# well-robotics/Decentralized_EKF_MHE

Measured on AMD Instinct MI355X. Metric: estimator-steps/sec (EKF+MHE, 20-step window), higher is better.
Workload: dtype f64

## Files before the change

### decentralized_ekf_mhe_amd/csrc/cfg.h

```cpp
#pragma once
#include "../../include/dekf.h"
#include "wave.h"

namespace dekf {

#ifndef DEKF_SOLVE_THREADS
#define DEKF_SOLVE_THREADS 256
#endif

#ifndef DEKF_QUEUE_MODE
#define DEKF_QUEUE_MODE 2
#endif
#define DEKF_R4_THREADS 192

constexpr int DEKF_PROF_SLOTS = 32;
constexpr double OSQP_INFTY = 1e30;
constexpr double RHO_MIN = 1e-6, RHO_MAX = 1e6, RHO_EQ_OVER_RHO_INEQ = 1e3, RHO_TOL = 1e-4;
constexpr double MIN_SCALING = 1e-4, MAX_SCALING = 1e4;

struct DevCfg {
    int B, L, nj, N, nm;
    int ft;
    int ns;
    int SV, SC;
    int ring;
    int wcap;
    int rec;
    int snap_len;
    int est_type;
    int marg_info;
    double dt;
    double hdt2, rho0c, inf_thr;
    int gws_wt;
    double C_p[3], C_accel[3], C_accel_bias[3], C_gyro[3];
    double C_enc_pos[DEKF_MAX_JOINTS], C_enc_vel[DEKF_MAX_JOINTS];
    double C_swing[3], Q_swing[3], Q_vo[3], Q_bias_dt2[3];
    double C_slide[3], Q_slide[3];
    double Q_prior[9], C_prior[9];
    double Q_foot_init[3], C_foot_init[3];
    double rho0, sigma, alpha, eps_abs, eps_rel;
    int max_iter, scaling, check_termination, adaptive_rho, adaptive_rho_interval;
    double adaptive_rho_tolerance;
    int polish, polish_refine_iter;
    int polish_accept_osqp;
    double delta;
    double ekf_dt, ekf_Cgyro[3], ekf_Caccel[3], ekf_Cvo[4], ekf_P0[4], ekf_q0[4];
    int ekf_hist;
// ... 75 lines not shown
        cf = o; o += m_pad;
        pol = o; o += 2 * K * ns + 5 * m_pad;
        WT = o; o += wt && !ft ? K * b2 : 0;
        o += wt && !ft ? 8 * 81 : 0;
        total = o;
    }
};

struct DevState {
    double *imu_t, *accel, *gyro, *p_foot, *J, *qdot, *contact, *quat;
    int* vo_flag;
    double *vo_tpre, *vo_tnow, *vo_dp;
    int* ekf_vo_flag;
    double *ekf_vo_t, *ekf_vo_q;
    double *ekf_q, *ekf_P, *ekf_hist;
    double *st_time, *st_R;
    int* st_dtime;
    double *rec, *Mp, *np_;
    double *Mp_next, *np_next;
    int* marg_tag;
    double* snap;
    double *wp, *wpt;
    int* wp_count;
    double* p_vo;
    int *vo_ins_idx, *vo_ins_dtime;
    double* gws;
    int* queue;
    double *kf_x, *kf_C;
    double *x_mhe, *v_b;
    int *status, *iters, *rho_updates;
    int* polish_status;
    double *pri_res, *dua_res;
    double* prof;
    double* warm = nullptr;
    int* warm_tag = nullptr;
    int* warm_used = nullptr;
};

}
```

### decentralized_ekf_mhe_amd/csrc/dekf_capi.hip

```cpp
#include <hip/hip_runtime.h>
#include <cstdlib>

#include <cstdio>
#include <cstring>
#include <string>
#include <vector>

#include "../../include/dekf.h"
#include "cfg.h"
#include "host_common.h"
#include "kf_core.h"
#include "mhe_assemble_core.h"
#include "mhe_direct_core.h"
#include "mhe_solve_core.h"

using namespace dekf;

extern "C" {
__global__ void k_ekf_tick(DevCfg c, DevState s, int count);
__global__ void k_mhe_initialize(DevCfg c, DevState s);
__global__ void k_mhe_assemble(DevCfg c, DevState s, int T, int pushes);
__global__ void k_mhe_marginalize_early(DevCfg c, DevState s, int T);
#define DEKF_SOLVE_KERNEL(NAME, ...)                                                   \
    __global__ void NAME(DevCfg c, DevState s, int kstart, int K, int gws_len);        \
// ... 437 lines not shown
    if (h->early_stream) { (void)hipStreamSynchronize(h->early_stream); (void)hipStreamDestroy(h->early_stream); }
    if (h->ev_asm_done) (void)hipEventDestroy(h->ev_asm_done);
    if (h->ev_early_done) (void)hipEventDestroy(h->ev_early_done);
    if (h->ev_early_mark) (void)hipEventDestroy(h->ev_early_mark);
    if (h->comm_stream) (void)hipStreamSynchronize(h->comm_stream);
    if (h->comm) rccl_destroy(h->comm);
    if (h->ev_vb_ready) (void)hipEventDestroy(h->ev_vb_ready);
    if (h->ev_ag_done) (void)hipEventDestroy(h->ev_ag_done);
    for (int i = 0; i < 2; ++i) if (h->ev_vb_read[i]) (void)hipEventDestroy(h->ev_vb_read[i]);
    if (h->comm_stream) (void)hipStreamDestroy(h->comm_stream);
    if (h->vb_snapshot) (void)hipFree(h->vb_snapshot);
    for (auto& v : h->ev) for (auto& pr : v) { (void)hipEventDestroy(pr.first); (void)hipEventDestroy(pr.second); }
    for (auto& pr : h->ev_pool) { (void)hipEventDestroy(pr.first); (void)hipEventDestroy(pr.second); }
    for (void* q : h->blocks) (void)hipFree(q);
    if (h->stage) (void)hipFree(h->stage);
    if (h->own_stream && h->stream) (void)hipStreamDestroy(h->stream);
    delete h;
    return DEKF_OK;
}

dekf_status dekf_reset(dekf_handle h) {
    if (!h) return fail(DEKF_ERR_INVALID, "null handle");
    HIPCHK(hipSetDevice(h->device));
    for (int i = 0; i < 2; ++i)
        if (h->solve_pending[i]) { HIPCHK(hipStreamWaitEvent(h->stream, h->ev_solve[i], 0)); h->solve_pending[i] = false; }
    for (int i = 0; i < DEKF_SNAP_SETS; ++i) h->snap_busy[i] = false;
    if (h->early_pending) { HIPCHK(hipStreamWaitEvent(h->stream, h->ev_early_done, 0)); h->early_pending = false; }
    for (int i = 0; i < 2; ++i)
        if (h->vb_read_pending[i]) { HIPCHK(hipStreamWaitEvent(h->stream, h->ev_vb_read[i], 0)); h->vb_read_pending[i] = false; }
    for (int i = 0; i < (h->pipelined ? 2 : 1); ++i) {
        k_reset_state<<<(h->c.B + 255) / 256, 256, 0, h->stream>>>(h->c, h->sp[i]);
        HIPCHK(hipGetLastError());
    }
    h->last_par = 0;
    h->ekf_count = 0;
    h->pushes = 0;
    h->next_T = 0;
    h->initialized = false;
    h->mhe_cov_valid = false;
    h->win_steps = 0;
    return DEKF_OK;
}

dekf_status dekf_sync(dekf_handle h) {
    if (!h) return fail(DEKF_ERR_INVALID, "null handle");
    HIPCHK(hipStreamSynchronize(h->stream));
    for (int i = 0; i < 2; ++i)
        if (h->solve_stream[i]) HIPCHK(hipStreamSynchronize(h->solve_stream[i]));
    if (h->comm_stream) HIPCHK(hipStreamSynchronize(h->comm_stream));
    if (h->early_stream) HIPCHK(hipStreamSynchronize(h->early_stream));
    return DEKF_OK;
}
int dekf_batch(dekf_handle h) { return h ? h->c.B : 0; }
void* dekf_stream(dekf_handle h) { return h ? (void*)h->stream : nullptr; }

dekf_status dekf_push_imu(dekf_handle h, const double* imu_time, const double* accel_b, const double* gyro_b, dekf_mem where) {
    if (!h) return fail(DEKF_ERR_INVALID, "null handle");
    size_t B = h->c.B;
    double* const dst[3] = {h->s.imu_t, h->s.accel, h->s.gyro};
    const double* const src[3] = {imu_time, accel_b, gyro_b};
    const size_t cnt[3] = {B, 3 * B, 3 * B};
    return put_many(h, 3, dst, src, cnt, where);
}

dekf_status dekf_push_leg(dekf_handle h, const double* p_imu_2_foot, const double* J_imu_2_foot, const double* joint_velocity,
                          const double* contact, dekf_mem where) {
// ... 608 lines not shown
```

### decentralized_ekf_mhe_amd/csrc/host_common.h

```cpp
#pragma once
#include <cmath>
#include <cstddef>
#include <cstring>

#include "cfg.h"
#include "ekf_core.h"

namespace dekf {

inline void default_params(dekf_params* p) {
    std::memset(p, 0, sizeof(*p));
    auto set3 = [](double* a, double x, double y, double z) { a[0] = x; a[1] = y; a[2] = z; };
    set3(p->p_init_std, 0.001, 0.001, 0.001);
    set3(p->v_init_std, 0.001, 0.001, 0.001);
    set3(p->foot_init_std, 0.001, 0.001, 0.001);
    set3(p->accel_bias_init_std, 0.0001, 0.0001, 0.0001);
    set3(p->p_process_std, 0.001, 0.001, 0.001);
    set3(p->accel_input_std, 0.025, 0.025, 0.02);
    set3(p->gyro_input_std, 0.03, 0.03, 0.03);
    set3(p->accel_bias_std, 0.07, 0.02, 0.03);
    p->quaternion_ib[0] = 1.0;
    set3(p->p_ib, 0.01592, 0.06659, 0.00617);
    p->num_legs = 4; p->joints_per_leg = 3; p->leg_odom_type = 0;
    for (int i = 0; i < DEKF_MAX_JOINTS; ++i) { p->joint_position_std[i] = 0.04; p->joint_velocity_std[i] = 0.22; }
// ... 85 lines not shown
    for (int i = 0; i < 4; ++i) {
        c.ekf_Cvo[i] = sq(p.ekf_vo_meas_std[i]);
        c.ekf_P0[i] = sq(p.ekf_init_std[i]);
        c.ekf_q0[i] = p.ekf_quaternion_init[i];
    }
    c.ekf_hist = p.ekf_history;
    return nullptr;
}

constexpr int DEKF_SNAP_SETS = 3;
template <class Alloc>
inline void alloc_state(const DevCfg& c, DevState& s, int solve_slots, Alloc alloc, int copies = 1) {
    const size_t B = (size_t)c.B, L = (size_t)c.L, nj = (size_t)c.nj;
    auto D = [&](size_t n) { return (double*)alloc(n * sizeof(double)); };
    auto I = [&](size_t n) { return (int*)alloc(n * sizeof(int)); };
    s.imu_t = D(B); s.accel = D(3 * B); s.gyro = D(3 * B);
    s.p_foot = D(3 * L * B); s.J = D(3 * L * nj * B); s.qdot = D(L * nj * B); s.contact = D(L * B);
    s.quat = D(4 * B);
    s.vo_flag = I(B); s.vo_tpre = D(B); s.vo_tnow = D(B); s.vo_dp = D(3 * B);
    s.ekf_vo_flag = I(B); s.ekf_vo_t = D(B); s.ekf_vo_q = D(4 * B);
    s.ekf_q = D(4 * B); s.ekf_P = D(16 * B); s.ekf_hist = D((size_t)c.ekf_hist * EKF_HIST_REC * B);
    s.st_time = D((size_t)c.ring * B); s.st_R = D((size_t)c.ring * 9 * B); s.st_dtime = I((size_t)c.ring * B);
    const size_t ns = (size_t)c.ns;
    s.rec = D((size_t)c.wcap * c.rec * B); s.Mp = D(ns * ns * B); s.np_ = D(ns * B);
    s.Mp_next = D(ns * ns * B); s.np_next = D(ns * B); s.marg_tag = I(B);
    s.snap = D((size_t)(copies > 1 ? DEKF_SNAP_SETS : 1) * c.snap_len * B);
    s.wp = D(12 * B); s.wpt = D(4 * B); s.wp_count = I(B);
    s.p_vo = D(3 * B); s.vo_ins_idx = I(B); s.vo_ins_dtime = I(B);
    Gws g;
    g.init(c.N, c.L, c.ft, c.gws_wt);
    const size_t cp = (size_t)copies;
    s.gws = D(cp * solve_slots * g.total);
    s.queue = I(cp * 2);
    s.kf_x = D(ns * B); s.kf_C = D(ns * ns * B);
    s.x_mhe = D(cp * ns * B); s.v_b = D(cp * 3 * B);
    s.status = I(cp * B); s.iters = I(cp * B); s.rho_updates = I(cp * B); s.polish_status = I(cp * B);
    s.pri_res = D(cp * B); s.dua_res = D(cp * B);
    s.prof = D(cp * DEKF_PROF_SLOTS * B);
}
inline DevState second_set(const DevCfg& c, const DevState& s, int solve_slots) {
    const size_t B = (size_t)c.B, ns = (size_t)c.ns;
    Gws g;
    g.init(c.N, c.L, c.ft, c.gws_wt);
    DevState t = s;
    t.gws += (size_t)solve_slots * g.total;
    t.queue += 2;
    t.x_mhe += ns * B; t.v_b += 3 * B;
    t.status += B; t.iters += B; t.rho_updates += B; t.polish_status += B;
    t.pri_res += B; t.dua_res += B;
    t.prof += DEKF_PROF_SLOTS * B;
    return t;
}

}
```

### decentralized_ekf_mhe_amd/csrc/kernels.hip

```cpp
#include <hip/hip_runtime.h>

#include "cfg.h"
#include "ekf_core.h"
#include "go1_kin.h"
#include "kf_core.h"
#include "mhe_assemble_core.h"
#include "mhe_direct_core.h"
#include "mhe_solve_core.h"

using namespace dekf;

#ifdef DEKF_BOUNDS
namespace dekf {
__device__ unsigned long long dekf_bounds_hits[4] = {0ull, 0ull, 0ull, 0ull};
}
extern "C" __global__ void k_bounds_selftest(double* a) {
    dekf::dptr p = DEKF_SPAN(a, 16);
    const double v = p[16];
    (p + 3)[13] = v + 1.0;
}
#endif

__device__ __forceinline__ void solve_queue_leave(const dekf::DevState& s) {
#if DEKF_QUEUE_MODE == 0
// ... 60 lines not shown
    int b = blockIdx.x * 64 + threadIdx.x;
    if (b < c.B) ekf_tick(c, s, b, count);
}

__global__ void __launch_bounds__(64) k_mhe_initialize(DevCfg c, DevState s) {
    extern __shared__ double lds[];
    assemble_initialize(c, s, blockIdx.x, lds);
    if (threadIdx.x == 0) { s.status[blockIdx.x] = DEKF_SOLVE_NONE; s.iters[blockIdx.x] = 0; }
}

#ifndef DEKF_ASM_WAVES
#define DEKF_ASM_WAVES 3
#endif
__global__ void __launch_bounds__(64, DEKF_ASM_WAVES) k_mhe_assemble(DevCfg c, DevState s, int T, int pushes) {
    extern __shared__ double lds[];
    assemble_update(c, s, blockIdx.x, T, pushes, lds);
}
__global__ void __launch_bounds__(64, DEKF_ASM_WAVES) k_mhe_marginalize_early(DevCfg c, DevState s, int T) {
    extern __shared__ double lds[];
    marginalize_early(c, s, blockIdx.x, T, lds);
}
#endif

#ifndef DEKF_SOLVE_MIN_WAVES
#define DEKF_SOLVE_MIN_WAVES 2
#endif
#define DEKF_SOLVE_BODY_(NAME, THREADS, WAVES, LOOP, ON, POLISH, WARM, ...)                                                   \
    __global__ void __launch_bounds__(THREADS, WAVES) NAME(DevCfg c, DevState s, int kstart, int K, int gws_len) {            \
        if constexpr (ON) {                                                                                                  \
        extern __shared__ double lds[];                                                                                      \
        __shared__ int next_instance;                                                                                        \
        double* gws = s.gws + (size_t)blockIdx.x * gws_len;                                                                  \
        DEKF_WG_TRACE_BEGIN                                                                                                  \
        LOOP(SolveEntry<POLISH, WARM>::template run<__VA_ARGS__>(c, s, b, kstart, K, lds, gws))                              \
        solve_queue_leave(s);                                                                                                \
        DEKF_WG_TRACE_END                                                                                                    \
        }                                                                                                                    \
    }
#define DEKF_SOLVE_STUB_(NAME) __global__ void NAME(DevCfg, DevState, int, int, int) {}
#define DEKF_WARM_TWIN_(ROLE) DEKF_WARM_TWIN_##ROLE
#ifdef DEKF_NO_POLISH_KERNELS
#define DEKF_SOLVE_KERNEL(NAME, ROLE, THREADS, WAVES, LOOP, ...)                                                              \
    DEKF_SOLVE_BODY_(NAME, THREADS, WAVES, LOOP, true, false, !DEKF_WARM_TWIN_(ROLE), __VA_ARGS__)                            \
    DEKF_SOLVE_STUB_(NAME##_pol)                                                                                             \
    DEKF_SOLVE_BODY_(NAME##_warm, THREADS, WAVES, LOOP, DEKF_WARM_TWIN_(ROLE), false, true, __VA_ARGS__)                      \
    DEKF_SOLVE_STUB_(NAME##_warm_pol)
#else
#define DEKF_SOLVE_KERNEL(NAME, ROLE, THREADS, WAVES, LOOP, ...)                                                              \
    DEKF_SOLVE_BODY_(NAME, THREADS, WAVES, LOOP, true, false, !DEKF_WARM_TWIN_(ROLE), __VA_ARGS__)                            \
    DEKF_SOLVE_BODY_(NAME##_pol, THREADS, WAVES, LOOP, true, true, !DEKF_WARM_TWIN_(ROLE), __VA_ARGS__)                       \
    DEKF_SOLVE_BODY_(NAME##_warm, THREADS, WAVES, LOOP, DEKF_WARM_TWIN_(ROLE), false, true, __VA_ARGS__)                      \
    DEKF_SOLVE_BODY_(NAME##_warm_pol, THREADS, WAVES, LOOP, DEKF_WARM_TWIN_(ROLE), true, true, __VA_ARGS__)
#endif
#ifdef DEKF_KSET_ONLY
#define DEKF_SOLVE_KERNEL_OFF(...)
#else
#define DEKF_SOLVE_KERNEL_OFF(NAME, ...) DEKF_SOLVE_STUB_(NAME) DEKF_SOLVE_STUB_(NAME##_pol) DEKF_SOLVE_STUB_(NAME##_warm) DEKF_SOLVE_STUB_(NAME##_warm_pol)
#endif
#include "solve_kernels.def"

#define DEKF_DIRECT_KERNEL(NAME, L, FT, NFIX)                                                                                 \
    __global__ void __launch_bounds__(64) NAME(DevCfg c, DevState s, int kstart, int K, double* cov) {                         \
        extern __shared__ double lds[];                                                                                      \
        direct_solve_t<L, FT>(c, s, blockIdx.x, kstart, K, lds, cov);                                                         \
    }                                                                                                                        \
    __global__ void __launch_bounds__(64) NAME##_smooth(DevCfg c, DevState s, int kstart, int K, double* cov, DirectWindow win) { \
        extern __shared__ double lds[];                                                                                      \
// ... 100 lines not shown
```

### decentralized_ekf_mhe_amd/csrc/mhe_admm_core.h

```cpp
#pragma once
#pragma clang fp contract(off)

template <class Q, class WF>
DEKF_FN double gather_pcol(const Q& q, int k, int a, WF w) {
    const bool hn = k < q.K - 1, hp = k > 0;
    const int kn = hn ? k : 0, kp = hp ? k - 1 : 0;
    const double n0 = w(q.ix.rd(kn, a)), n1 = w(q.ix.rv(kn, a)), p0 = w(q.ix.rd(kp, a)), p1 = w(q.ix.rv(kp, a));
    double g = (hn ? n0 + n1 : 0.0) - (hp ? p0 + p1 : 0.0);
    if constexpr (Q::FOOT) {
#pragma unroll
        for (int leg = 0; leg < Q::LEGS; ++leg) g -= w(q.ix.rm(k, 3 * leg + a));
    }
    return g;
}
template <class Q, class WF>
DEKF_FN double gather_fcol(const Q& q, int k, int la, WF w) {
    const bool hn = k < q.K - 1, hp = k > 0;
    const int kn = hn ? k : 0, kp = hp ? k - 1 : 0;
    const double m0 = w(q.ix.rm(k, la)), n0 = w(q.ix.rd(kn, 9 + la)), p0 = w(q.ix.rd(kp, 9 + la));
    return m0 + (hn ? n0 : 0.0) - (hp ? p0 : 0.0);
}
template <class Q, class WF>
DEKF_FN double gather_vcol(const Q& q, int k, int a, WF w) {
    constexpr int L = Q::LEGS;
// ... 1477 lines not shown
    else if constexpr (XKIND == 1) { x.r[0] = q.ix.rm(k, a); x.r[1] = q.ix.rd(kn, 3 + a); x.r[2] = q.ix.rd(kn, a); x.r[3] = q.ix.rd(kp, 3 + a); }
    else { x.r[0] = q.ix.rd(kn, 6 + a); x.r[1] = 3 * kn + a; x.r[2] = q.ix.rd(kp, 6 + a); x.r[3] = 0; }
    x.dv = q.D[k * (21 + 3 * Q::LEGS) + j];
    const double qv = (q.tmp + TmpMap<9>::QSL)[j];
    x.q0 = k == 0 ? qv : 0.0;
}
template <int XKIND, class Q>
DEKF_FN void xcols_regs_tile(Q& q, const XcolRegs<XKIND>& x, double sigma) {
    if (!x.valid) return;
    cdptr at = q.at;
    const double xv = q.xb[x.i];
    double g;
    if constexpr (XKIND == 0) {
        const double n0 = at[x.r[0]], n1 = at[x.r[1]], p0 = at[x.r[2]], p1 = at[x.r[3]];
        g = (x.hn ? n0 + n1 : 0.0) - (x.hp ? p0 + p1 : 0.0);
    } else if constexpr (XKIND == 1) {
        const double n0 = at[x.r[1]], n1 = at[x.r[2]], p0 = at[x.r[3]];
        double gm = 0.0;
#pragma unroll
        for (int leg = 0; leg < Q::LEGS; ++leg) gm += at[x.r[0] + 3 * leg];
        g = gm + (x.hn ? fma(q.c.dt, n1, n0) : 0.0) - (x.hp ? p0 : 0.0);
    } else {
        const double n0 = at[x.r[0]], n1 = q.gb[x.r[1]], p0 = at[x.r[2]];
        g = (x.hn ? n0 - n1 : 0.0) - (x.hp ? p0 : 0.0);
    }
    q.xs[x.i] = fma(x.dv, g, fma(sigma, xv, -x.q0));
}
template <int NF, class Q>
DEKF_FN void admm_chunk_r3(Q& q, int iters, double alpha, double sigma) {
    constexpr int L = Q::LEGS, SV = 21 + 3 * L;
    static_assert(3 * NF <= 64 && 2 * (NF - 1) <= 64, "one tile per kind");
    static_assert(NF * L <= 64 || (NF * L - 64) + 2 * (NF - 1) <= 64, "the Meas blocks beyond 64 fit the VO / bias wavefront");
    const int w = __builtin_amdgcn_readfirstlane(DEKF_LANE() >> 6), lane = DEKF_LANE() & 63;
#if defined(DEKF_PROFILE_TL)
#define DEKF_R3_T(var) const long long var = clock64()
#else
#define DEKF_R3_T(var) ((void)0)
#endif
    if (w == 0) {
        DEKF_SYNC();
        DEKF_PROF_MARK(q, 14);
        for (int it = 0; it < iters; ++it) {
            DEKF_R3_T(t0);
            DEKF_SYNC();
            DEKF_R3_T(t1);
            __builtin_amdgcn_s_setprio(3);
            sweeps_one_wave<NF>(q, alpha, lane);
            __builtin_amdgcn_s_setprio(0);
#if defined(DEKF_PROFILE_TL)
            __builtin_amdgcn_s_waitcnt(0);
#endif
            DEKF_R3_T(t2);
            DEKF_SYNC();
            DEKF_SYNC();
            DEKF_R3_T(t3);
            DEKF_TL_ADD(q, 0, t1, t2);
            DEKF_TL_ADD(q, 4, t2, t3);
            DEKF_TL_ADD(q, 8, t0, t1);
        }
    } else {
        auto worker = [&](auto tag) {
            constexpr int KIND = decltype(tag)::value;
            RowRegsT<KIND> t;
            row_regs_load<KIND>(q, lane, sigma, t);
            DEKF_SYNC();
            constexpr int xkind = KIND == 0 ? 1 : (KIND == 1 ? 2 : 0);
            const bool cold = q.cold;
            XcolRegs<xkind> xc;
            xcols_regs_load<xkind>(q, lane, xc);
            for (int it = 0; it < iters; ++it) {
                DEKF_R3_T(t0);
                xcols_regs_tile<xkind>(q, xc, sigma);
#if defined(DEKF_PROFILE_TL)
                __builtin_amdgcn_s_waitcnt(0);
#endif
                DEKF_R3_T(t1);
                DEKF_SYNC();
                DEKF_SYNC();
                DEKF_R3_T(t2);
                if constexpr (KIND == 1) __builtin_amdgcn_s_setprio(2);
                row_regs_iter<KIND>(q, t, alpha, sigma, cold && it == 0 && !q.polishing());
                if constexpr (KIND == 1) __builtin_amdgcn_s_setprio(0);
#if defined(DEKF_PROFILE_TL)
                __builtin_amdgcn_s_waitcnt(0);
#endif
                DEKF_R3_T(t3);
                DEKF_SYNC();
                DEKF_TL_ADD(q, w, t0, t1);
                DEKF_TL_ADD(q, 4 + w, t2, t3);
                DEKF_TL_ADD(q, 8 + w, t1, t2);
            }
            row_regs_store<KIND>(q, t);
        };
        if (w == 1) worker(std::integral_constant<int, 0>{});
        else if (w == 2) worker(std::integral_constant<int, 1>{});
        else worker(std::integral_constant<int, 2>{});
    }
#undef DEKF_R3_T
    DEKF_PROF_MARK(q, 9);
    DEKF_SYNC();
    q.cold = false;
    DEKF_PROF_MARK(q, 15);
}

template <int NF, class Q>
DEKF_FN void admm_chunk_r4(Q& q, int iters, double alpha, double sigma) {
    constexpr int L = Q::LEGS;
    static_assert(3 * NF <= 64 && 2 * (NF - 1) <= 64, "one tile per kind");
    static_assert(NF * L <= 64 || (NF * L - 64) + 2 * (NF - 1) <= 64, "the Meas blocks beyond 64 fit the VO / bias tile");
    const int w = __builtin_amdgcn_readfirstlane(DEKF_LANE() >> 6), lane = DEKF_LANE() & 63;
#if defined(DEKF_PROFILE_TL)
#define DEKF_R4_T(var) const long long var = clock64()
#else
#define DEKF_R4_T(var) ((void)0)
#endif
    if (w == 0) {
        DEKF_SYNC();
        DEKF_PROF_MARK(q, 14);
        for (int it = 0; it < iters; ++it) {
            DEKF_R4_T(t0);
            DEKF_SYNC();
            DEKF_R4_T(t1);
            __builtin_amdgcn_s_setprio(3);
            sweeps_one_wave<NF>(q, alpha, lane);
            __builtin_amdgcn_s_setprio(0);
#if defined(DEKF_PROFILE_TL)
            __builtin_amdgcn_s_waitcnt(0);
#endif
// ... 498 lines not shown
            const int e = td * 64 + lane;
            if (e >= NM * K) return;
            const int k = e / NM, la = e - NM * k, j = 9 + la, i = k * SV + j;
            const double d = D[i], qv = k == 0 ? qsl[j] : 0.0;
            const double g = gather_fcol(q, k, la, wy);
            double Px = 0.0;
            if (k == 0) {
                for (int t = 0; t < NS; ++t) Px += (j <= t ? q.Mp[NS * j + t] : q.Mp[NS * t + j]) * xd[t];
                Px *= cc * d;
            }
            const double Aty = d * g, dr = qv + Px + Aty, di = rcp_fast(d);
            if (rv) rv->rxb[NS * k + j] = -dr;
            acc[6] = dmax(acc[6], fabs(dr) * di);
            acc[7] = dmax(acc[7], fabs(qv) * di);
            acc[8] = dmax(acc[8], fabs(Aty) * di);
            acc[9] = dmax(acc[9], fabs(Px) * di);
            acc[10] = dmax(acc[10], fabs(dr));
            acc[11] = dmax(acc[11], fabs(qv));
            acc[12] = dmax(acc[12], fabs(Aty));
            acc[13] = dmax(acc[13], fabs(Px));
        }
    });
    DEKF_PROF_MARK(q, 21);
#if defined(DEKF_PROFILE) && defined(DEKF_PROFILE_RESID2) && DEKF_DEVICE_BUILD
    __builtin_amdgcn_s_waitcnt(0);
    const long long trs1 = clock64();
#endif
    wave_max_n<14>(acc);
    group_combine<14, false>(acc);
#if defined(DEKF_PROFILE) && defined(DEKF_PROFILE_RESID2) && DEKF_DEVICE_BUILD
    {
        const long long trs2 = clock64();
        const int w_ = DEKF_LANE() >> 6;
        if ((DEKF_LANE() & 63) == 0) { q.prof[24 + w_] += (double)(trs1 - trs0); q.prof[28 + w_] += (double)(trs2 - trs1); }
    }
#endif
#pragma unroll
    for (int r = 0; r < 6; ++r) ra[r] = acc[r];
#pragma unroll
    for (int r = 0; r < 8; ++r) va[r] = acc[6 + r];
}
#pragma clang fp contract(fast)
```

### decentralized_ekf_mhe_amd/csrc/mhe_solve_core.h

```cpp
#pragma once
#include "cfg.h"
#include "mhe_assemble_core.h"
#include "smallmat.h"

namespace dekf {

#if defined(DEKF_PROFILE) && defined(DEKF_PROFILE_TL) && DEKF_DEVICE_BUILD
#define DEKF_PROF_MARK(q, sec) ((void)0)
#define DEKF_TL_ADD(q, slot, t0, t1)                                            \
    do {                                                                        \
        if ((DEKF_LANE() & 63) == 0) (q).prof[slot] += (double)((t1) - (t0));   \
    } while (0)
#elif defined(DEKF_PROFILE) && DEKF_DEVICE_BUILD
#define DEKF_TL_ADD(q, slot, t0, t1) ((void)0)
#define DEKF_PROF_MARK(q, sec)                                                  \
    do {                                                                        \
        if (DEKF_LANE() == 0) {                                                 \
            long long now_ = clock64();                                         \
            (q).prof[sec] += (double)(now_ - (q).prof_last);                    \
            (q).prof_last = now_;                                               \
        }                                                                       \
    } while (0)
#else
#define DEKF_PROF_MARK(q, sec) ((void)0)
#define DEKF_TL_ADD(q, slot, t0, t1) ((void)0)
#endif

DEKF_HD constexpr int mid_block(int K) { return (K - 1) / 2; }
constexpr int SWS = 25;
constexpr int SOLVE_TMP = 344;
template <int NS>
struct TmpMap {
    static constexpr int QSL = NS == 9 ? 162 : 0;
    static constexpr int FAIL = NS == 9 ? 172 : NS;
    static constexpr int SIDE0 = NS == 9 ? 0 : NS + 8;
    static constexpr int SIDE1 = NS == 9 ? 176 : SIDE0 + NS * NS + 2 * NS;
    static constexpr int LEN = NS == 9 ? SOLVE_TMP : SIDE1 + NS * NS + 2 * NS + 8;
};
DEKF_HD constexpr int solve_tmp_len(int ns) { return ns == 9 ? SOLVE_TMP : 2 * (ns * ns + 2 * ns) + ns + 16; }

struct SolveLayout {
    int n_pad, m_pad, K, ns;
    int vec;
    int resident;
    DEKF_HD void init(int N, int L, int ft = 0) {
        int nm = 3 * L;
        K = N;
        ns = 9 + (ft ? nm : 0);
        n_pad = N * (2 * ns + nm + 3);
        m_pad = N * (nm + ns + 3);
        vec = 2 * n_pad + 4 * m_pad + 2 * ns * N + solve_tmp_len(ns);
        resident = n_pad + 2 * m_pad + 3 * N + N * (6 * L + SWS + 6 + (ft ? 6 * L : 0)) + N * 2 * ns * ns + 9 * N;
    }
    DEKF_HD bool factor_in_lds() const { return (size_t)(vec + resident) * 8 <= 80 * 1024; }
    DEKF_HD bool pa_in_lds() const { return factor_in_lds() && (n_pad + 2 * m_pad >= (K - 1) * ns * ns); }
#ifndef DEKF_R3_WAVES
#define DEKF_R3_WAVES 3
#endif
#ifndef DEKF_R3_PA_LDS
// ... 35 lines not shown
        return with >= 1 && with == (wgs_per_cu((size_t)vec * 8) < 2 ? wgs_per_cu((size_t)vec * 8) : 2);
    }
    DEKF_HD size_t lds_bytes() const { return (size_t)(factor_in_lds() ? vec + resident : (gg_consts_in_lds() ? vec + gg_consts() : vec)) * 8; }
};

template <int L, int FT = 0>
struct IdxT {
    static constexpr int nm = 3 * L, NS = 9 + 3 * L * FT, SV = 2 * NS + 3 + 3 * L, SC = NS + 3 + 3 * L;
    DEKF_FN static int x(int k, int j) { return k * SV + j; }
    DEKF_FN static int v(int k, int r) { return k * SV + NS + r; }
    DEKF_FN static int w(int k, int r) { return k * SV + NS + nm + r; }
    DEKF_FN static int c(int k, int a) { return k * SV + 2 * NS + nm + a; }
    int rdb, rvb;
    DEKF_FN explicit IdxT(int K) : rdb(K * nm), rvb(K * nm + NS * (K - 1)) {}
    DEKF_FN int rm(int k, int r) const { return k * nm + r; }
    DEKF_FN int rd(int k, int r) const { return rdb + NS * k + r; }
    DEKF_FN int rv(int k, int a) const { return rvb + 3 * k + a; }
};

DEKF_FN double mul_rounded(double a, double b) {
    double p = a * b;
#if DEKF_DEVICE_BUILD
    asm volatile("" : "+v"(p));
#endif
    return p;
}

template <int L, int NF = 0, bool FLDS = true, int FT = 0, bool R3_ = false, bool POLISH_ = false, bool R4_ = false>
struct SolveCtx {
    static constexpr bool R4 = R4_;
    static constexpr int WAVES = R4_ ? 3 : 4;
    static constexpr bool POLISH = POLISH_;
    static constexpr bool R3 = R3_;
    static constexpr int LEGS = L;
    static constexpr int NFIXED = NF;
    static constexpr bool FACTOR_LDS = FLDS;
    static constexpr int FOOT = FT;
    static constexpr int NS = 9 + 3 * L * FT, NS2 = NS * NS;
    const DevCfg& c;
    const DevState& s;
    int b, K, kstart, n, m;
    IdxT<L, FT> ix;
    dptr x, z, y, xt, zt, at, xs, xd, tmp;
    dptr xb;
    dptr Dxb;
    dptr sx, sy, sz;
    bool cold;
    dptr cf;
    dptr gb;
    dptr D, E, lo, hi, Sv, Sw, Sc, Sinv, Wk, R;
    dptr Sf;
    dptr Wm, Wd, Wc, PA;
    dptr WT;
    dptr Wf;
    cdptr Mp, np;
    cdptr vo;
    double cc;
    double rho;
    int lane0;
    double sigma_pol;
    bool zlo;
    DEKF_FN double sigma() const { if constexpr (POLISH) return zlo ? sigma_pol : c.sigma; else return c.sigma; }
    DEKF_FN bool polishing() const { if constexpr (POLISH) return zlo; else return false; }
    dptr pol;
    dptr Pst;
    bool staged;
// ... 377 lines not shown
            for (int t = 0; t < 6; ++t) p6[t] = q6[t];
#pragma unroll
            for (int a = 0; a < 3; ++a)
                vv3[a] = dmax(fabs(p6[symidx(0, a, 3)] * dout[0]), dmax(fabs(p6[1 < a ? symidx(1, a, 3) : symidx(a, 1, 3)] * dout[1]), fabs(p6[symidx(a, 2, 3)] * dout[2]))) * dout[a];
        }
#pragma unroll
        for (int a = 0; a < 3; ++a) { Ew[r0 + a] = eo[a]; Dw[sv0 + a] = dout[a]; pc[sv0 + a] = vv3[a]; }
        return vv3[0] + vv3[1] + vv3[2];
    };
    auto fused_x0 = [&](int tile, int lane, cdptr Dw) -> double {
        int kind, k, sub;
        if (tile < ntm + ntp + 2 * ntd || tile >= ntm + ntp + 2 * ntd + 3 * ntx) return 0.0;
        if (!decode(tile, lane, kind, k, sub) || k != 0) return 0.0;
        const int j = 3 * (kind - 4) + sub;
        const double dj = Dw[j];
        double mj[9], dt9[9], v = 0.0;
#pragma unroll
        for (int t = 0; t < 9; ++t) { mj[t] = symget(Mst, j, t, 9); dt9[t] = Dw[t]; }
#pragma unroll
        for (int t = 0; t < 9; ++t) v = dmax(v, fabs(dj * mj[t] * dt9[t]));
        pc[j] = v;
        return v;
    };
#endif
    wtiles(ntiles, [&](int tile, int lane) { (void)adopt(tile, lane); });
    DEKF_SYNC();
    DEKF_PROF_MARK(q, 16);
    double gq[NS];
#pragma unroll
    for (int j = 0; j < NS; ++j) gq[j] = g[j];
#if DEKF_DEVICE_BUILD
    {
        dptr Dr = D, Er = E, Dw = Dn, Ew = En;
        const int rz_lane = DEKF_LANE() & 63, rz_wave = __builtin_amdgcn_readfirstlane(DEKF_LANE() >> 6), rz_nw = DEKF_NLANES() > WAVE ? DEKF_NLANES() >> 6 : 1;
        (void)rz_lane; (void)rz_wave; (void)rz_nw;
        for (int it = 0; it < q.c.scaling; ++it) {
            const double cc = q.cc;
            double psum = 0.0;
#if defined(DEKF_PROFILE) && defined(DEKF_PROFILE_RUIZ)
            const long long tr0 = clock64();
#endif
            constexpr bool RZ3 = Q::WAVES == 3;
            constexpr int RZ_PW[4] = {0, Q::LEGS == 4 ? 1 : 2, Q::LEGS == 4 ? 2 : 1, Q::LEGS == 4 ? 1 : 0};
            const int rz_nrow = ntm + ntp + 2 * ntd + ntf;
            auto rz_phys = [&](int t) { return t < rz_nrow ? RZ_PW[t & 3] : 2 - (t - rz_nrow) % 3; };
            double pv[4] = {0.0, 0.0, 0.0, 0.0};
            if constexpr (RZ3) {
                for (int t = 0; t < ntiles; ++t) {
                    if (rz_phys(t) != rz_wave) continue;
                    const double f = fused(t, rz_lane, cc, Dr, Er, Dw, Ew);
                    const int v = t & 3;
                    pv[0] += v == 0 ? f : 0.0; pv[1] += v == 1 ? f : 0.0; pv[2] += v == 2 ? f : 0.0; pv[3] += v == 3 ? f : 0.0;
                }
            } else {
                for (int t = rz_wave; t < ntiles; t += rz_nw) psum += fused(t, rz_lane, cc, Dr, Er, Dw, Ew);
            }
#if defined(DEKF_PROFILE) && defined(DEKF_PROFILE_RUIZ)
            long long tr1 = 0, tr2 = 0;
#endif
            {
                const int wv = __builtin_amdgcn_readfirstlane(DEKF_LANE() >> 6), ln = DEKF_LANE() & 63;
                dptr part = q.tmp + 176 + 4 * (it & 1);
                if constexpr (RZ3) {
#pragma unroll
                    for (int v = 0; v < 4; ++v)
                        if (RZ_PW[v] == wv) { const double sv_ = wave_sum_dpp(pv[v]); if (ln == 0) part[v] = sv_; }
                } else {
                    psum = wave_sum_dpp(psum);
                    if (ln == 0) part[wv] = psum;
                }
#if defined(DEKF_PROFILE) && defined(DEKF_PROFILE_RUIZ)
                __builtin_amdgcn_s_waitcnt(0);
                tr1 = clock64();
#endif
                DEKF_SYNC();
#if defined(DEKF_PROFILE) && defined(DEKF_PROFILE_RUIZ)
                tr2 = clock64();
#endif
                const int j = ln < NS ? ln : NS - 1;
                const double dj = Dw[j];
                double v = 0.0;
                if constexpr (FT) {
                    for (int t = 0; t < NS; ++t) v = dmax(v, fabs(dj * symget(Mst, j, t, NS) * Dw[t]));
                } else {
                    double mj[9], dt9[9];
#pragma unroll
                    for (int t = 0; t < 9; ++t) { mj[t] = symget(Mst, j, t, 9); dt9[t] = Dw[t]; }
#pragma unroll
                    for (int t = 0; t < 9; ++t) v = dmax(v, fabs(dj * mj[t] * dt9[t]));
                }
                const int cpos = j < 3 ? 1 : (j < 6 ? 0 : 2);
                const int otile = j < 9 ? ntm + ntp + 2 * ntd + cpos * ntx : ntm + ntp + 2 * ntd + 3 * ntx + ntf;
                if (ln < NS && (RZ3 ? rz_phys(otile) : (otile & (DEKF_NLANES() / WAVE - 1))) == wv) pc[j] = v;
                const double x0 = wave_sum_dpp(ln < NS ? v : 0.0);
                const int nw = RZ3 ? 4 : DEKF_NLANES() >> 6;
                double tot = part[0];
                for (int i = 1; i < nw; ++i) tot += part[i];
                psum = tot + x0;
            }
#if defined(DEKF_PROFILE) && defined(DEKF_PROFILE_RUIZ)
            {
                const long long tr3 = clock64();
                const int w_ = DEKF_LANE() >> 6;
                if ((DEKF_LANE() & 63) == 0) { q.prof[24 + w_] += (double)(tr1 - tr0); q.prof[28 + w_] += (double)(tr2 - tr1); q.prof[17 + (w_ & 1)] += 0.5 * (double)(tr3 - tr2); }
            }
#endif
            psum *= cc;
            double qn = 0.0;
#pragma unroll
            for (int j = 0; j < NS; ++j) qn = dmax(qn, fabs(cc * Dw[j] * gq[j]));
            double ct = 1.0 / limit_scaling(dmax(psum / uni((double)n), limit_scaling(qn)));
            q.cc = uni_pin(cc * ct);
            dptr t0 = Dr; Dr = Dw; Dw = t0;
            dptr t1 = Er; Er = Ew; Ew = t1;
        }
        if (Dr != D) {
            DEKF_SYNC();
            cdptr Ds = Dr, Es = Er;
            wfor(n + m, [&](int e) { if (e < n) D[e] = Ds[e]; else E[e - n] = Es[e - n]; });
        }
        DEKF_SYNC();
        return;
    }
#endif
    for (int it = 0; it < q.c.scaling; ++it) {
        const double cc = q.cc;
        wtiles(ntiles, [&](int tile, int lane) { equil(tile, lane, cc); });
        DEKF_SYNC();
        double psum = 0.0;
        wtiles(ntiles, [&](int tile, int lane) { psum += adopt(tile, lane); });
        psum = wave_sum(psum);
        group_combine<1, true>(&psum);
        psum *= cc;
        double qn = 0.0;
#pragma unroll
        for (int j = 0; j < NS; ++j) qn = dmax(qn, fabs(cc * D[j] * gq[j]));
        double ct = 1.0 / limit_scaling(dmax(psum / uni((double)n), limit_scaling(qn)));
// ... 560 lines not shown
#undef DEKF_GJ_UPD
#undef DEKF_GJ_OWN
#undef DEKF_GJ_PIVOT
#undef DEKF_GJ_DPP
        const bool inv_lane = icol;
        const int jc = ic;
        if (inv_lane) {
#pragma unroll
            for (int i = 0; i < 9; ++i) {
                q.Sinv[k * 81 + 9 * i + jc] = a[i];
                if (wmode == 0) ts[9 * i + jc] = a[i];
            }
        }
        if (ccol) {
#pragma unroll
            for (int t = 0; t < 9; ++t) q.Wk[kw * 81 + 9 * cidx + t] = a[t];
            if constexpr (!W_DIRECT) {
#pragma unroll
                for (int t = 0; t < 9; ++t) q.WT[kw * 81 + 9 * t + cidx] = a[t];
            }
            if constexpr (!W_DIRECT) {
#pragma unroll
                for (int t = 0; t < 9; ++t) two[9 * cidx + t] = a[t];
            }
        }
        wave_sync();
        return good;
    };
    dptr fail = q.tmp + 172;
    if (DEKF_LANE() == 0) *fail = 0.0;
    DEKF_SYNC();
    two_waves(
        [&] {
            bool g = true;
            if constexpr (W_DIRECT) {
                for (int k = 0; k < mid; ++k) g = factor_block(k, k > 0, false, 1, q.tmp, q.tmp + 81, q.tmp + 81, q.tmp + 81) && g;
            } else {
                SOps nx;
                if (mid > 0) s_ops_load(0, false, nx);
                for (int k = 0; k < mid; ++k) {
                    const SOps cu = nx;
                    if (k + 1 < mid) s_ops_load(k + 1, true, nx);
                    g = factor_block(k, k > 0, false, 1, q.tmp, q.tmp + 81, q.tmp + 81, q.tmp + 81, &cu) && g;
                }
            }
            if (!g && (DEKF_LANE() & 63) == 0) *fail = 1.0;
        },
        [&] {
            bool g = true;
            if constexpr (W_DIRECT) {
                for (int k = K - 1; k > mid; --k) g = factor_block(k, false, k < K - 1, 2, q.tmp + 176, q.tmp + 257, q.tmp + 257, q.tmp + 257) && g;
            } else {
                SOps nx;
                if (K - 1 > mid) s_ops_load(K - 1, true, nx);
                for (int k = K - 1; k > mid; --k) {
                    const SOps cu = nx;
                    if (k - 1 > mid) s_ops_load(k - 1, false, nx);
                    g = factor_block(k, false, k < K - 1, 2, q.tmp + 176, q.tmp + 257, q.tmp + 257, q.tmp + 257, &cu) && g;
                }
            }
            if (!g && (DEKF_LANE() & 63) == 0) *fail = 1.0;
        });
    DEKF_SYNC();
    DEKF_PROF_MARK(q, 22);
    two_waves(
        [&] {
            bool g = factor_block(mid, mid > 0, mid < K - 1, 0, q.tmp, q.tmp + 81, q.tmp + 257, q.tmp + 81);
            if (!g && (DEKF_LANE() & 63) == 0) *fail = 1.0;
            if constexpr (Q::NFIXED >= 4 && Q::NFIXED % 2 == 0) {
                if (K == Q::NFIXED) {
                    const int lane = DEKF_LANE() & 63;
                    cdptr P11 = q.tmp;
                    dptr P12 = q.tmp + 81;
                    cdptr Wh = q.Wk + mid * 81;
                    for (int pp = lane; pp < 81; pp += WAVE) {
                        const int i = pp / 9, j = pp - 9 * i;
                        double s0 = P11[9 * i] * Wh[j] + P11[9 * i + 3] * Wh[27 + j] + P11[9 * i + 6] * Wh[54 + j];
                        double s1 = P11[9 * i + 1] * Wh[9 + j] + P11[9 * i + 4] * Wh[36 + j] + P11[9 * i + 7] * Wh[63 + j];
                        double s2 = P11[9 * i + 2] * Wh[18 + j] + P11[9 * i + 5] * Wh[45 + j] + P11[9 * i + 8] * Wh[72 + j];
                        P12[pp] = -(s0 + (s1 + s2));
                    }
                    wave_sync();
                    double p22[2];
                    for (int pp = lane, n = 0; pp < 81; pp += WAVE, ++n) {
                        const int i = pp / 9, j = pp - 9 * i;
                        double s0 = Wh[i] * P12[j] + Wh[27 + i] * P12[27 + j] + Wh[54 + i] * P12[54 + j];
                        double s1 = Wh[9 + i] * P12[9 + j] + Wh[36 + i] * P12[36 + j] + Wh[63 + i] * P12[63 + j];
                        double s2 = Wh[18 + i] * P12[18 + j] + Wh[45 + i] * P12[45 + j] + Wh[72 + i] * P12[72 + j];
                        p22[n] = q.Sinv[(mid + 1) * 81 + pp] - (s0 + (s1 + s2));
                    }
                    wave_sync();
                    for (int pp = lane, n = 0; pp < 81; pp += WAVE, ++n) {
                        q.Wk[mid * 81 + pp] = P12[pp];
                        if constexpr (!W_DIRECT) q.WT[mid * 81 + 9 * (pp % 9) + pp / 9] = P12[pp];
// ... 417 lines not shown
            if constexpr (FT) q.Wf = DEKF_SPAN(wb + NH * 6 * L + NH * 30, NH * 6 * L);
        }
    }
    q.pol = DEKF_SPAN(raw_of(gws) + g.pol, 2 * NH * NS + 5 * lay.m_pad);
    q.n = (K - 1) * IdxT<L, FT>::SV + NS + IdxT<L, FT>::nm;
    q.m = (K - 1) * IdxT<L, FT>::SC + IdxT<L, FT>::nm;
    {
        const double* sn = s.snap + (size_t)c.snap_len * b;
        q.Mp = DEKF_CSPAN(sn, NS2);
        q.np = DEKF_CSPAN(sn + NS2, NS);
        q.vo = DEKF_CSPAN(sn + NS2 + NS, 4 * c.wcap);
    }
    q.cc = 1.0;
    q.lane0 = DEKF_LANE() & 63;
    q.sigma_pol = c.delta;
    q.zlo = false;
    q.Pst = DEKF_SPAN(raw_of(q.Sinv), 2 * NH * NS2);
    q.staged = false;
    const int n = q.n, m = q.m;
    const auto& ix = q.ix;
    SolveInfo info{0, DEKF_SOLVE_MAX_ITER, 0, 0.0, 0.0, c.rho0};
#if defined(DEKF_BOUNDS) && DEKF_DEVICE_BUILD
    const unsigned long long bounds_hits0 = *(volatile unsigned long long*)&dekf_bounds_hits[0];
#endif

    q.prof = DEKF_SPAN(s.prof + DEKF_PROF_SLOTS * (size_t)b, DEKF_PROF_SLOTS);
#if defined(DEKF_PROFILE) && DEKF_DEVICE_BUILD
    q.prof_last = clock64();
    const long long prof_t0 = q.prof_last;
    const long long prof_w0 = wall_clock64();
    if (DEKF_LANE() == 0)
        for (int i = 0; i < DEKF_PROF_SLOTS; ++i) q.prof[i] = 0.0;
#endif
    wfor(K * 9, [&](int e) { q.R[e] = ld_stream(q.rec(e / 9), Rec::R + e % 9); });
    if constexpr (R3 && !FACTOR_LDS) {
        double* const ob = raw_of(q.xb);
        q.xt = DEKF_SPAN(ob, lay.n_pad);
        q.zt = DEKF_SPAN(ob + lay.n_pad, lay.m_pad);
        if (c.scaling > 0) solve_scale(q);
        else { wfor(n + m, [&](int e) { if (e < n) q.D[e] = 1.0; else q.E[e - n] = 1.0; }); }
        q.zt = nullptr; q.xt = nullptr;
        wfor(K * NS, [&](int e) { q.xb[e] = 0.0; });
    } else if constexpr (R3) {
        constexpr int PSL = NFIX * (6 * L + 27) + NS * (NS + 1) / 2;
        dptr xg = q.x, ztg = nullptr;
        double* const sb = raw_of(q.Sinv);
        q.x = DEKF_SPAN(sb + PSL, lay.n_pad);
        q.zt = DEKF_SPAN(sb + PSL + lay.n_pad, lay.m_pad);
        q.xt = DEKF_SPAN(sb + PSL + lay.n_pad + lay.m_pad, lay.n_pad);
        dptr Dg = q.D, Eg = q.E;
        if constexpr (R4) {
            q.D = DEKF_SPAN(raw_of(q.xb), lay.n_pad);
            q.E = DEKF_SPAN(raw_of(q.xb) + lay.n_pad, lay.m_pad);
        }
        if (c.scaling > 0) solve_scale(q);
        else { wfor(n + m, [&](int e) { if (e < n) q.D[e] = 1.0; else q.E[e - n] = 1.0; }); }
        if constexpr (R4) {
            cdptr Dl = q.D, El = q.E;
            wfor(n + m, [&](int e) { if (e < n) Dg[e] = Dl[e]; else Eg[e - n] = El[e - n]; });
            q.D = Dg; q.E = Eg;
        }
        q.x = xg; q.zt = ztg; q.xt = nullptr;
        wfor(K * NS, [&](int e) { q.xb[e] = 0.0; });
    } else {
    if (c.scaling > 0) solve_scale(q);
    else { wfor(n + m, [&](int e) { if (e < n) q.D[e] = 1.0; else q.E[e - n] = 1.0; }); }
    }
// ... 210 lines not shown
    if (*(volatile unsigned long long*)&dekf_bounds_hits[0] != bounds_hits0) info.status = DEKF_SOLVE_NUMERIC;
#endif
    if (DEKF_LANE() == 0) {
        const double p_opti[3] = {0.016041, 0.089061, 0.0579875};
        double wxp[3], t[3], vb[3];
        double gy[3], Rl[9];
        for (int a = 0; a < 3; ++a) gy[a] = rT[Rec::GY + a];
        for (int a = 0; a < 9; ++a) Rl[a] = rT[Rec::R + a];
        cross3(gy, p_opti, wxp);
        for (int a = 0; a < 3; ++a) t[a] = xT[3 + a] + wxp[a];
        mv3(Rl, t, vb);
        for (int j = 0; j < NS; ++j) s.x_mhe[NS * (size_t)b + j] = xT[j];
        for (int a = 0; a < 3; ++a) s.v_b[3 * (size_t)b + a] = vb[a];
        s.status[b] = info.status;
        s.iters[b] = info.iters;
        s.rho_updates[b] = info.rho_updates;
        s.polish_status[b] = info.polished;
        s.pri_res[b] = info.pri_res;
        s.dua_res[b] = info.dua_res;
    }
    DEKF_SYNC();
#if defined(DEKF_PROFILE) && DEKF_DEVICE_BUILD
    DEKF_PROF_MARK(q, 12);
    if (DEKF_LANE() == 0) { q.prof[13] = (double)(clock64() - prof_t0); q.prof[23] = (double)(wall_clock64() - prof_w0); }
#endif
    return info;
}
template <bool POLISH, bool WARM>
struct SolveEntry {
    template <int L, bool FACTOR_LDS, bool PA_LDS, int NFIX = 0, int FT = 0, bool R3 = false>
    DEKF_FN static SolveInfo run(const DevCfg& c, const DevState& s, int b, int kstart, int K, dptr lds, dptr gws) {
        return solve_window_t<POLISH, L, FACTOR_LDS, PA_LDS, NFIX, FT, R3, WARM>(c, s, b, kstart, K, lds, gws);
    }
};
template <int L, bool FACTOR_LDS, bool PA_LDS, int NFIX = 0, int FT = 0, bool R3 = false>
DEKF_FN SolveInfo solve_window(const DevCfg& c, const DevState& s, int b, int kstart, int K, dptr lds, dptr gws) {
    return solve_window_t<false, L, FACTOR_LDS, PA_LDS, NFIX, FT, R3>(c, s, b, kstart, K, lds, gws);
}

}
```

Baseline: 2.136 million.

## Remap wavefront roles by SIMD occupancy so heavy work lands on uncontended SIMDs

Each solve workgroup reads its hardware SIMD and CU ids, records per-SIMD occupancy in a global atomic counter array, and classifies which of its wavefronts sit on a SIMD not shared with another workgroup. The R3 row-assembly workers and the Ruiz scaling reduction then swap wavefront roles so the heaviest role runs on the free SIMD. The aim is to cut SIMD contention between co-resident workgroups. It adds global atomics at kernel entry and exit, a getreg-based placement query, a reset memset, and by-class profiling hooks.

```diff
diff --git a/decentralized_ekf_mhe_amd/csrc/cfg.h b/decentralized_ekf_mhe_amd/csrc/cfg.h
--- a/decentralized_ekf_mhe_amd/csrc/cfg.h
+++ b/decentralized_ekf_mhe_amd/csrc/cfg.h
@@ -13,6 +13,10 @@
 #endif
 #define DEKF_R4_THREADS 192
 
+#ifndef DEKF_SIMD_SPLIT
+#define DEKF_SIMD_SPLIT 6
+#endif
+constexpr int DEKF_SIMD_OCC_WORDS = 4096;
 constexpr int DEKF_PROF_SLOTS = 32;
 constexpr double OSQP_INFTY = 1e30;
 constexpr double RHO_MIN = 1e-6, RHO_MAX = 1e6, RHO_EQ_OVER_RHO_INEQ = 1e3, RHO_TOL = 1e-4;
@@ -154,6 +158,7 @@
     int* polish_status;
     double *pri_res, *dua_res;
     double* prof;
+    int* simd_occ;
     double* warm = nullptr;
     int* warm_tag = nullptr;
     int* warm_used = nullptr;
diff --git a/decentralized_ekf_mhe_amd/csrc/dekf_capi.hip b/decentralized_ekf_mhe_amd/csrc/dekf_capi.hip
--- a/decentralized_ekf_mhe_amd/csrc/dekf_capi.hip
+++ b/decentralized_ekf_mhe_amd/csrc/dekf_capi.hip
@@ -493,6 +493,7 @@
         k_reset_state<<<(h->c.B + 255) / 256, 256, 0, h->stream>>>(h->c, h->sp[i]);
         HIPCHK(hipGetLastError());
     }
+    HIPCHK(hipMemsetAsync(h->s.simd_occ, 0, DEKF_SIMD_OCC_WORDS * sizeof(int), h->stream));
     h->last_par = 0;
     h->ekf_count = 0;
     h->pushes = 0;
diff --git a/decentralized_ekf_mhe_amd/csrc/host_common.h b/decentralized_ekf_mhe_amd/csrc/host_common.h
--- a/decentralized_ekf_mhe_amd/csrc/host_common.h
+++ b/decentralized_ekf_mhe_amd/csrc/host_common.h
@@ -141,6 +141,7 @@
     const size_t cp = (size_t)copies;
     s.gws = D(cp * solve_slots * g.total);
     s.queue = I(cp * 2);
+    s.simd_occ = I(DEKF_SIMD_OCC_WORDS);
     s.kf_x = D(ns * B); s.kf_C = D(ns * ns * B);
     s.x_mhe = D(cp * ns * B); s.v_b = D(cp * 3 * B);
     s.status = I(cp * B); s.iters = I(cp * B); s.rho_updates = I(cp * B); s.polish_status = I(cp * B);
diff --git a/decentralized_ekf_mhe_amd/csrc/kernels.hip b/decentralized_ekf_mhe_amd/csrc/kernels.hip
--- a/decentralized_ekf_mhe_amd/csrc/kernels.hip
+++ b/decentralized_ekf_mhe_amd/csrc/kernels.hip
@@ -116,7 +116,9 @@
         __shared__ int next_instance;                                                                                        \
         double* gws = s.gws + (size_t)blockIdx.x * gws_len;                                                                  \
         DEKF_WG_TRACE_BEGIN                                                                                                  \
+        SolveEntry<POLISH, WARM>::template enter<__VA_ARGS__>(s);                                                            \
         LOOP(SolveEntry<POLISH, WARM>::template run<__VA_ARGS__>(c, s, b, kstart, K, lds, gws))                              \
+        SolveEntry<POLISH, WARM>::template leave<__VA_ARGS__>(s);                                                            \
         solve_queue_leave(s);                                                                                                \
         DEKF_WG_TRACE_END                                                                                                    \
         }                                                                                                                    \
diff --git a/decentralized_ekf_mhe_amd/csrc/mhe_admm_core.h b/decentralized_ekf_mhe_amd/csrc/mhe_admm_core.h
--- a/decentralized_ekf_mhe_amd/csrc/mhe_admm_core.h
+++ b/decentralized_ekf_mhe_amd/csrc/mhe_admm_core.h
@@ -1533,6 +1533,8 @@
     static_assert(3 * NF <= 64 && 2 * (NF - 1) <= 64, "one tile per kind");
     static_assert(NF * L <= 64 || (NF * L - 64) + 2 * (NF - 1) <= 64, "the Meas blocks beyond 64 fit the VO / bias wavefront");
     const int w = __builtin_amdgcn_readfirstlane(DEKF_LANE() >> 6), lane = DEKF_LANE() & 63;
+    int role = w;
+    if constexpr (Q::PLACED && (DEKF_SIMD_SPLIT & 2) != 0) role = SimdPlace::virtual_wave();
 #if defined(DEKF_PROFILE_TL)
 #define DEKF_R3_T(var) const long long var = clock64()
 #else
@@ -1590,11 +1592,15 @@
                 DEKF_TL_ADD(q, w, t0, t1);
                 DEKF_TL_ADD(q, 4 + w, t2, t3);
                 DEKF_TL_ADD(q, 8 + w, t1, t2);
+#if defined(DEKF_PROFILE_TL)
+                DEKF_CLS_ADD(q, 4, t2, t3);
+                DEKF_CLS_ADD(q, 5, t0, t1);
+#endif
             }
             row_regs_store<KIND>(q, t);
         };
-        if (w == 1) worker(std::integral_constant<int, 0>{});
-        else if (w == 2) worker(std::integral_constant<int, 1>{});
+        if (role == 1) worker(std::integral_constant<int, 0>{});
+        else if (role == 2) worker(std::integral_constant<int, 1>{});
         else worker(std::integral_constant<int, 2>{});
     }
 #undef DEKF_R3_T
@@ -2159,7 +2165,12 @@
     {
         const long long trs2 = clock64();
         const int w_ = DEKF_LANE() >> 6;
+#if defined(DEKF_PROFILE_BYCLASS)
+        (void)w_; (void)trs2;
+        DEKF_CLS_ADD(q, 2, trs0, trs1);
+#else
         if ((DEKF_LANE() & 63) == 0) { q.prof[24 + w_] += (double)(trs1 - trs0); q.prof[28 + w_] += (double)(trs2 - trs1); }
+#endif
     }
 #endif
 #pragma unroll
diff --git a/decentralized_ekf_mhe_amd/csrc/mhe_solve_core.h b/decentralized_ekf_mhe_amd/csrc/mhe_solve_core.h
--- a/decentralized_ekf_mhe_amd/csrc/mhe_solve_core.h
+++ b/decentralized_ekf_mhe_amd/csrc/mhe_solve_core.h
@@ -5,7 +5,20 @@
 
 namespace dekf {
 
-#if defined(DEKF_PROFILE) && defined(DEKF_PROFILE_TL) && DEKF_DEVICE_BUILD
+#if defined(DEKF_PROFILE) && defined(DEKF_PROFILE_BYCLASS) && DEKF_DEVICE_BUILD
+#define DEKF_PROF_MARK(q, sec) ((void)0)
+#define DEKF_TL_ADD(q, slot, t0, t1) ((void)0)
+#define DEKF_CLS_ADD(q, phase, t0, t1)                                                                       \
+    do {                                                                                                     \
+        if (DEKF_PROFILE_BYCLASS == (phase) && (DEKF_LANE() & 63) == 0) {                                    \
+            const int w_ = DEKF_LANE() >> 6;                                                                 \
+            const int cl_ = SimdPlace::wave_class(w_);                                                       \
+            const int s_ = w_ == 0 ? 9 : 3 * (w_ - 1) + (cl_ == 0 ? 3 : cl_) - 1;                            \
+            (q).prof[s_] += (double)((t1) - (t0));                                                           \
+            (q).prof[w_ == 0 ? 10 : 14 + s_] += 1.0;                                                         \
+        }                                                                                                    \
+    } while (0)
+#elif defined(DEKF_PROFILE) && defined(DEKF_PROFILE_TL) && DEKF_DEVICE_BUILD
 #define DEKF_PROF_MARK(q, sec) ((void)0)
 #define DEKF_TL_ADD(q, slot, t0, t1)                                            \
     do {                                                                        \
@@ -25,6 +38,83 @@
 #define DEKF_PROF_MARK(q, sec) ((void)0)
 #define DEKF_TL_ADD(q, slot, t0, t1) ((void)0)
 #endif
+#ifndef DEKF_CLS_ADD
+#define DEKF_CLS_ADD(q, phase, t0, t1) ((void)0)
+#endif
+
+#if DEKF_DEVICE_BUILD
+#if defined(DEKF_PROFILE) && defined(DEKF_PROFILE_BYCLASS)
+#define DEKF_SIMD_PLACE_ON 1
+#else
+#define DEKF_SIMD_PLACE_ON (DEKF_SIMD_SPLIT != 0)
+#endif
+struct SimdPlace {
+    static DEKF_FN int* lds() {
+        __shared__ int place[8];
+        return place;
+    }
+    static DEKF_FN void enter(const DevState& s) {
+        int* p = lds();
+        const unsigned hw = __builtin_amdgcn_s_getreg((31 << 11) | (0 << 6) | 4);
+        const unsigned xcc = __builtin_amdgcn_s_getreg((3 << 11) | (0 << 6) | 20) & 0xf;
+        const int simd = (hw >> 4) & 3;
+        if ((threadIdx.x & 63) == 0) p[threadIdx.x >> 6] = simd;
+        if (threadIdx.x == 0) {
+            const int cu = (int)((xcc << 8) | (((hw >> 13) & 7) << 5) | (((hw >> 12) & 1) << 4) | ((hw >> 8) & 0xf));
+            p[4] = cu;
+            p[5] = 0;
+            atomicAdd(s.simd_occ + cu, 1 << (8 * simd));
+        }
+        __syncthreads();
+    }
+    static DEKF_FN void leave(const DevState& s) {
+        const int* p = lds();
+        if (threadIdx.x == 0) atomicSub(s.simd_occ + p[4], 1 << (8 * p[0]));
+    }
+    static DEKF_FN int begin(const DevState& s) {
+        return DEKF_LANE() == 0 ? __hip_atomic_load(s.simd_occ + lds()[4], __ATOMIC_RELAXED, __HIP_MEMORY_SCOPE_AGENT) : 0;
+    }
+    static DEKF_FN int classify(int word, const int* p) {
+        int cnt[4], seen = 0, total = 0;
+        bool ok = true;
+#pragma unroll
+        for (int i = 0; i < 4; ++i) { cnt[i] = (word >> (8 * i)) & 0xff; ok = ok && cnt[i] <= 1; total += cnt[i]; seen |= 1 << p[i]; }
+        ok = ok && seen == 0xf && ((word >> (8 * p[0])) & 0xff) == 1 && total >= 2;
+        int pk = 0, free_w = 0;
+#pragma unroll
+        for (int wi = 0; wi < 3; ++wi) {
+            const int w = wi == 0 ? 2 : (wi == 1 ? 1 : 3);
+            const bool fr = ok && ((word >> (8 * p[w])) & 0xff) == 0;
+            if (fr && free_w == 0) free_w = w;
+            pk |= (ok ? (fr ? 1 : 2) : 3) << (4 + 2 * w);
+        }
+        return pk | free_w;
+    }
+    static DEKF_FN void publish(int word) {
+        int* p = lds();
+        if (DEKF_LANE() == 0) p[5] = classify(word, p);
+    }
+    static DEKF_FN int packed() { return __builtin_amdgcn_readfirstlane(lds()[5]); }
+    static DEKF_FN int free_wave() { return packed() & 3; }
+    static constexpr int virt(int f, int w) { return f == 0 || f == 2 ? w : (w == f ? 2 : (w == 2 ? f : w)); }
+    static DEKF_FN int virtual_wave() {
+        const int f = free_wave(), w = __builtin_amdgcn_readfirstlane(DEKF_LANE() >> 6);
+        return virt(f, w);
+    }
+    static DEKF_FN int wave_class(int w) { return (packed() >> (4 + 2 * w)) & 3; }
+};
+constexpr bool simd_virt_is_permutation() {
+    for (int f = 0; f < 4; ++f) {
+        int seen = 0;
+        for (int w = 0; w < 4; ++w) seen |= 1 << SimdPlace::virt(f, w);
+        if (seen != 0xf || SimdPlace::virt(f, 0) != 0 || (f != 0 && SimdPlace::virt(f, f) != 2)) return false;
+    }
+    return true;
+}
+static_assert(simd_virt_is_permutation(), "SimdPlace::virt: a permutation of the wavefronts 1..3 for every chain-free wavefront");
+#else
+#define DEKF_SIMD_PLACE_ON 0
+#endif
 
 DEKF_HD constexpr int mid_block(int K) { return (K - 1) / 2; }
 constexpr int SWS = 25;
@@ -126,6 +216,7 @@
     static constexpr int WAVES = R4_ ? 3 : 4;
     static constexpr bool POLISH = POLISH_;
     static constexpr bool R3 = R3_;
+    static constexpr bool PLACED = DEKF_SIMD_PLACE_ON && R3_ && FLDS && !R4_;
     static constexpr int LEGS = L;
     static constexpr int NFIXED = NF;
     static constexpr bool FACTOR_LDS = FLDS;
@@ -569,7 +660,10 @@
 #if DEKF_DEVICE_BUILD
     {
         dptr Dr = D, Er = E, Dw = Dn, Ew = En;
-        const int rz_lane = DEKF_LANE() & 63, rz_wave = __builtin_amdgcn_readfirstlane(DEKF_LANE() >> 6), rz_nw = DEKF_NLANES() > WAVE ? DEKF_NLANES() >> 6 : 1;
+        constexpr bool RZ_PLACED = Q::PLACED && (DEKF_SIMD_SPLIT & 4) != 0;
+        int rz_wave = __builtin_amdgcn_readfirstlane(DEKF_LANE() >> 6);
+        if constexpr (RZ_PLACED) rz_wave = SimdPlace::virtual_wave();
+        const int rz_lane = DEKF_LANE() & 63, rz_nw = DEKF_NLANES() > WAVE ? DEKF_NLANES() >> 6 : 1;
         (void)rz_lane; (void)rz_wave; (void)rz_nw;
         for (int it = 0; it < q.c.scaling; ++it) {
             const double cc = q.cc;
@@ -596,7 +690,7 @@
             long long tr1 = 0, tr2 = 0;
 #endif
             {
-                const int wv = __builtin_amdgcn_readfirstlane(DEKF_LANE() >> 6), ln = DEKF_LANE() & 63;
+                const int wv = RZ_PLACED ? rz_wave : __builtin_amdgcn_readfirstlane(DEKF_LANE() >> 6), ln = DEKF_LANE() & 63;
                 dptr part = q.tmp + 176 + 4 * (it & 1);
                 if constexpr (RZ3) {
 #pragma unroll
@@ -639,7 +733,12 @@
             {
                 const long long tr3 = clock64();
                 const int w_ = DEKF_LANE() >> 6;
+#if defined(DEKF_PROFILE_BYCLASS)
+                (void)tr3; (void)w_; (void)tr2;
+                DEKF_CLS_ADD(q, 1, tr0, tr1);
+#else
                 if ((DEKF_LANE() & 63) == 0) { q.prof[24 + w_] += (double)(tr1 - tr0); q.prof[28 + w_] += (double)(tr2 - tr1); q.prof[17 + (w_ & 1)] += 0.5 * (double)(tr3 - tr2); }
+#endif
             }
 #endif
             psum *= cc;
@@ -1266,6 +1365,9 @@
     DEKF_SYNC();
     two_waves(
         [&] {
+#if defined(DEKF_PROFILE) && defined(DEKF_PROFILE_BYCLASS)
+            const long long tl0 = clock64();
+#endif
             bool g = true;
             if constexpr (W_DIRECT) {
                 for (int k = 0; k < mid; ++k) g = factor_block(k, k > 0, false, 1, q.tmp, q.tmp + 81, q.tmp + 81, q.tmp + 81) && g;
@@ -1279,8 +1381,14 @@
                 }
             }
             if (!g && (DEKF_LANE() & 63) == 0) *fail = 1.0;
+#if defined(DEKF_PROFILE) && defined(DEKF_PROFILE_BYCLASS)
+            DEKF_CLS_ADD(q, 3, tl0, clock64());
+#endif
         },
         [&] {
+#if defined(DEKF_PROFILE) && defined(DEKF_PROFILE_BYCLASS)
+            const long long tl0 = clock64();
+#endif
             bool g = true;
             if constexpr (W_DIRECT) {
                 for (int k = K - 1; k > mid; --k) g = factor_block(k, false, k < K - 1, 2, q.tmp + 176, q.tmp + 257, q.tmp + 257, q.tmp + 257) && g;
@@ -1294,6 +1402,9 @@
                 }
             }
             if (!g && (DEKF_LANE() & 63) == 0) *fail = 1.0;
+#if defined(DEKF_PROFILE) && defined(DEKF_PROFILE_BYCLASS)
+            DEKF_CLS_ADD(q, 3, tl0, clock64());
+#endif
         });
     DEKF_SYNC();
     DEKF_PROF_MARK(q, 22);
@@ -1777,7 +1888,15 @@
     if (DEKF_LANE() == 0)
         for (int i = 0; i < DEKF_PROF_SLOTS; ++i) q.prof[i] = 0.0;
 #endif
-    wfor(K * 9, [&](int e) { q.R[e] = ld_stream(q.rec(e / 9), Rec::R + e % 9); });
+#if DEKF_DEVICE_BUILD
+    int simd_word = 0;
+    if constexpr (decltype(q)::PLACED) simd_word = SimdPlace::begin(s);
+#endif
+    wfor_nosync(K * 9, [&](int e) { q.R[e] = ld_stream(q.rec(e / 9), Rec::R + e % 9); });
+#if DEKF_DEVICE_BUILD
+    if constexpr (decltype(q)::PLACED) SimdPlace::publish(simd_word);
+#endif
+    DEKF_SYNC();
     if constexpr (R3 && !FACTOR_LDS) {
         double* const ob = raw_of(q.xb);
         q.xt = DEKF_SPAN(ob, lay.n_pad);
@@ -2054,6 +2173,16 @@
     DEKF_FN static SolveInfo run(const DevCfg& c, const DevState& s, int b, int kstart, int K, dptr lds, dptr gws) {
         return solve_window_t<POLISH, L, FACTOR_LDS, PA_LDS, NFIX, FT, R3, WARM>(c, s, b, kstart, K, lds, gws);
     }
+#if DEKF_DEVICE_BUILD
+    template <int L, bool FACTOR_LDS, bool PA_LDS, int NFIX = 0, int FT = 0, bool R3 = false>
+    DEKF_FN static void enter(const DevState& s) {
+        if constexpr (DEKF_SIMD_PLACE_ON && R3 && FACTOR_LDS && PA_LDS) SimdPlace::enter(s);
+    }
+    template <int L, bool FACTOR_LDS, bool PA_LDS, int NFIX = 0, int FT = 0, bool R3 = false>
+    DEKF_FN static void leave(const DevState& s) {
+        if constexpr (DEKF_SIMD_PLACE_ON && R3 && FACTOR_LDS && PA_LDS) SimdPlace::leave(s);
+    }
+#endif
 };
 template <int L, bool FACTOR_LDS, bool PA_LDS, int NFIX = 0, int FT = 0, bool R3 = false>
 DEKF_FN SolveInfo solve_window(const DevCfg& c, const DevState& s, int b, int kstart, int K, dptr lds, dptr gws) {
```

Measured after the change: 2.152 million, median of 6. About the same (+0.7%).
